# dmosopt/dmosopt

Measured on AMD Instinct MI355X. Metric: MO-ASMO epoch time (GP fit + 200-gen NSGA2), ZDT1 d=30, lower is better.
Workload: dtype fp32; 1 GPU; model=GPR-Matern52 surrogate + NSGA2, global_batch=200, parallelism=replicated-moea+sharded-gp dp1, population_size=200, archive_size=300

## Files before the change

dmosopt_amd/ops/hip/moea_device.h:

```cpp
#pragma once

#include "common.h"
#include <math.h>

__device__ __forceinline__ void sbx_children(float a, float b, float beta,
                                             float lo, float hi, float* c1,
                                             float* c2) {
  const float x1 = 0.5f * fmaf(-beta, a, fmaf(beta, b, a + b));
  const float x2 = 0.5f * fmaf(beta, a, fmaf(-beta, b, a + b));
  *c1 = fminf(fmaxf(x1, lo), hi);
  *c2 = fminf(fmaxf(x2, lo), hi);
}

__device__ __forceinline__ float mutated_child(float p, float delta, float lo,
                                               float hi) {
  const float v = fmaf(hi - lo, delta, p);
  return fminf(fmaxf(v, lo), hi);
}

template <typename PoolIdx>
__device__ __forceinline__ void variation_event_gene(
    const float* __restrict__ src, const PoolIdx* pool_row,
    const long long* __restrict__ ci, const long long* __restrict__ mi,
    const long long* __restrict__ p1, const long long* __restrict__ p2,
    const long long* __restrict__ im, const float* __restrict__ di_c,
    const float* __restrict__ di_m, const float* __restrict__ lo,
    const float* __restrict__ hi, float* __restrict__ out, int ev, int g,
    int C, int d, float mutation_rate, unsigned long long seed_sbx,
    unsigned long long seed_mut) {
  if (ev < C) {
    long long r1 = p1[ev], r2 = p2[ev];
    if (pool_row) { r1 = (long long)pool_row[r1]; r2 = (long long)pool_row[r2]; }
    const float a = src[r1 * d + g];
    const float b = src[r2 * d + g];
    const Philox4 r = philox4x32(seed_sbx, (unsigned long long)ev * d + g);
    const float u = u01(r.c0);
    const float e = 1.f / (di_c[g] + 1.f);
    const float beta = (u <= 0.5f) ? __powf(2.f * u, e)
                                   : __powf(1.f / (2.f * (1.f - u)), e);
    float c1, c2;
    sbx_children(a, b, beta, lo[g], hi[g], &c1, &c2);
    out[ci[2 * ev] * d + g] = c1;
    out[ci[2 * ev + 1] * d + g] = c2;
  } else {
    const int m = ev - C;
    long long r0 = im[m];
    if (pool_row) r0 = (long long)pool_row[r0];
    const float p = src[r0 * d + g];
    const Philox4 ph =
        philox4x32(seed_mut ^ 0x5deece66dULL, (unsigned long long)m * d + g);
    const float u = u01(ph.c0);
    const float e = 1.f / (di_m[g] + 1.f);
    const float delta = (u < mutation_rate)
                            ? __powf(2.f * u, e) - 1.f
                            : 1.f - __powf(2.f * (1.f - u), e);
    out[mi[m] * d + g] = mutated_child(p, delta, lo[g], hi[g]);
  }
}

__device__ __forceinline__ void crowding_gaps(const float* vals,
                                              const int* idxs, float* out,
                                              int N, int tid, int nthreads) {
  const float l = vals[0];
  const float h = vals[N - 1];
  float s = h - l;
  if (!(s > 0.f) || !isfinite(s)) s = 1.f;
  for (int i = tid; i < N; i += nthreads) {
    float d = (i == 0 || i == N - 1) ? 1.f : (vals[i + 1] - vals[i - 1]) / s;
    if (isnan(d)) d = 0.f;
    out[idxs[i]] = d;
  }
}

__device__ __forceinline__ void crowding_sort_gaps(float* vals, int* idxs,
                                                   float* out, int N,
                                                   int npow2, int tid,
                                                   int nthreads,
                                                   bool active = true) {
  for (int ksz = 2; ksz <= npow2; ksz <<= 1) {
    for (int jsz = ksz >> 1; jsz > 0; jsz >>= 1) {
      for (int i = tid; active && i < npow2; i += nthreads) {
        const int ixj = i ^ jsz;
        if (ixj > i) {
          const bool up = ((i & ksz) == 0);
          const bool swap = up ? (vals[i] > vals[ixj]) : (vals[i] < vals[ixj]);
          if (swap) {
            float tv = vals[i]; vals[i] = vals[ixj]; vals[ixj] = tv;
            int tixx = idxs[i]; idxs[i] = idxs[ixj]; idxs[ixj] = tixx;
          }
        }
      }
      __syncthreads();
    }
  }
  if (active) crowding_gaps(vals, idxs, out, N, tid, nthreads);
}

__device__ __forceinline__ long long rank_crowd_key(long long rank, float d) {
  if (isnan(d)) d = 0.f;
  const unsigned int b = __float_as_uint(d);
  const unsigned int asc = (b & 0x80000000u) ? ~b : (b | 0x80000000u);
  return (rank << 32) | (long long)(0xFFFFFFFFu - asc);
}

__device__ __forceinline__ void key_idx_sort(long long* keys, int* idxs, int M,
                                             int tid, int nthreads) {
  for (int k = 2; k <= M; k <<= 1) {
    for (int j = k >> 1; j > 0; j >>= 1) {
      for (int i = tid; i < M; i += nthreads) {
        const int ixj = i ^ j;
        if (ixj > i) {
          const bool up = ((i & k) == 0);
          const long long ka = keys[i], kb = keys[ixj];
          const int ia = idxs[i], ib = idxs[ixj];
          const bool gt = (ka > kb) || (ka == kb && ia > ib);
          if (gt == up) {
            keys[i] = kb; keys[ixj] = ka;
            idxs[i] = ib; idxs[ixj] = ia;
          }
        }
      }
      __syncthreads();
    }
  }
}
```

dmosopt_amd/ops/hip/moea_ops.hip:

```cpp

#include "common.h"
#include "launchers.h"
#include "moea_device.h"
#include <math.h>
#include <algorithm>

#define TOUR_TPB 256
#define TOUR_NMAX 2048

template <int TPB, bool COUNT>
__device__ __forceinline__ const int* tournament_order(
    const long long* __restrict__ rank, long long* key, int* idx, float* gkey,
    int* unsorted, int N, int npow2, float log1mp, unsigned long long seed) {
  const int tid = threadIdx.x;
  if (tid == 0) { unsorted[0] = 0; unsorted[1] = 0; }
  __syncthreads();
  for (int i = tid; i < npow2; i += TPB) {
    key[i] = (i < N) ? (rank[i] * (long long)N + i) : 0x7FFFFFFFFFFFFFFFLL;
    idx[i] = i;
    if (i + 1 < N && rank[i] > rank[i + 1]) atomicOr(&unsorted[0], 1);
  }
  __syncthreads();
  if (unsorted[0])
  for (int ks = 2; ks <= npow2; ks <<= 1) {
    for (int js = ks >> 1; js > 0; js >>= 1) {
      for (int i = tid; i < npow2; i += TPB) {
        const int ixj = i ^ js;
        if (ixj > i) {
          const bool up = ((i & ks) == 0);
          if (up ? (key[i] > key[ixj]) : (key[i] < key[ixj])) {
            long long tk = key[i]; key[i] = key[ixj]; key[ixj] = tk;
            int ti = idx[i]; idx[i] = idx[ixj]; idx[ixj] = ti;
          }
        }
      }
      __syncthreads();
    }
  }
  for (int i = tid; i < npow2; i += TPB) {
    if (i < N) {
      Philox4 r = philox4x32(seed, (unsigned long long)i);
      const float u = u01(r.c0);
      gkey[i] = (float)i * log1mp - logf(-logf(u));
    } else {
      gkey[i] = -INFINITY;
    }
  }
  __syncthreads();
  if (COUNT) {
    int* sel = (int*)key;
    bool tie = false;
    for (int i = tid; i < N; i += TPB) {
      const float gi = gkey[i];
      int pos = 0;
#pragma unroll 8
      for (int j = 0; j < N; ++j) {
        const float gj = gkey[j];
        pos += (gj > gi || (gj == gi && j < i)) ? 1 : 0;
        tie |= (gj == gi && j != i);
      }
      tie |= (gi != gi);
      sel[pos] = idx[i];
    }
    if (tie) atomicOr(&unsorted[1], 1);
    __syncthreads();
    if (!unsorted[1]) return sel;
  }
  for (int ks = 2; ks <= npow2; ks <<= 1) {
    for (int js = ks >> 1; js > 0; js >>= 1) {
      for (int i = tid; i < npow2; i += TPB) {
        const int ixj = i ^ js;
        if (ixj > i) {
          const bool up = ((i & ks) == 0);
          if (up ? (gkey[i] < gkey[ixj]) : (gkey[i] > gkey[ixj])) {
            float tg = gkey[i]; gkey[i] = gkey[ixj]; gkey[ixj] = tg;
            int ti = idx[i]; idx[i] = idx[ixj]; idx[ixj] = ti;
          }
        }
      }
      __syncthreads();
    }
  }
  return idx;
}

template <int TPB>
__global__ __launch_bounds__(TPB) void tournament_kernel(
    const float* __restrict__ population, const long long* __restrict__ rank,
    float* __restrict__ pool, long long* __restrict__ pool_idx, int N, int d,
    int poolsize, int npow2, float log1mp, unsigned long long seed) {
  extern __shared__ char sh_raw[];
  long long* key = (long long*)sh_raw;
  int* idx = (int*)(key + npow2);
  float* gkey = (float*)(idx + npow2);
  __shared__ int unsorted[2];
  const int tid = threadIdx.x;
  tournament_order<TPB, false>(rank, key, idx, gkey, unsorted, N, npow2,
                               log1mp, seed);
  for (int j = tid; j < poolsize; j += TPB) pool_idx[j] = idx[j];
  __syncthreads();
  for (long long t = tid; t < (long long)poolsize * d; t += TPB) {
    const int r = (int)(t / d), c = (int)(t % d);
    pool[t] = population[(long long)idx[r] * d + c];
  }
}

template <int TPB>
__global__ __launch_bounds__(TPB) void spawn_fused_kernel(
    const float* __restrict__ population, const long long* __restrict__ rank,
    int N, int d, int npow2, float log1mp, unsigned long long seed_t,
    const long long* __restrict__ ci, const long long* __restrict__ mi,
    const long long* __restrict__ p1, const long long* __restrict__ p2,
    const long long* __restrict__ im, const float* __restrict__ di_c,
    const float* __restrict__ di_m, const float* __restrict__ lo,
    const float* __restrict__ hi, float* __restrict__ out, int C, int M,
    float mutation_rate, unsigned long long seed_sbx,
    unsigned long long seed_mut) {
  extern __shared__ char sh_raw[];
  long long* key = (long long*)sh_raw;
  int* idx = (int*)(key + npow2);
  float* gkey = (float*)(idx + npow2);
  __shared__ int unsorted[2];
  const int* pool_row = tournament_order<TPB, true>(
      rank, key, idx, gkey, unsorted, N, npow2, log1mp, seed_t);
  const int total = (C + M) * d;
  for (int t = blockIdx.x * TPB + threadIdx.x; t < total; t += gridDim.x * TPB)
    variation_event_gene<int>(population, pool_row, ci, mi, p1, p2, im, di_c, di_m,
                              lo, hi, out, t / d, t % d, C, d, mutation_rate,
                              seed_sbx, seed_mut);
}

extern "C" int launch_tournament(const float* population, const long long* rank,
                                 float* pool, long long* pool_idx, int N,
                                 int d, int poolsize, float log1mp,
                                 unsigned long long seed, hipStream_t stream) {
  int npow2 = 1;
  while (npow2 < N) npow2 <<= 1;
  if (npow2 > TOUR_NMAX) return -1;
  const size_t lds = (size_t)npow2 * (8 + 4 + 4);
  if (npow2 > 512)
    hipLaunchKernelGGL(tournament_kernel<1024>, dim3(1), dim3(1024), lds,
                       stream, population, rank, pool, pool_idx, N, d,
                       poolsize, npow2, log1mp, seed);
  else
    hipLaunchKernelGGL(tournament_kernel<TOUR_TPB>, dim3(1), dim3(TOUR_TPB),
                       lds, stream, population, rank, pool, pool_idx, N, d,
                       poolsize, npow2, log1mp, seed);
  return 0;
}

extern "C" int launch_spawn_fused(
    const float* population, const long long* rank, int N, int d, int poolsize,
    float log1mp, unsigned long long seed_t, const long long* ci,
    const long long* mi, const long long* p1, const long long* p2,
    const long long* im, const float* di_c, const float* di_m, const float* lo,
    const float* hi, float* out, int C, int M, float mutation_rate,
    unsigned long long seed_sbx, unsigned long long seed_mut,
    hipStream_t stream) {
  int npow2 = 1;
  while (npow2 < N) npow2 <<= 1;
  if (npow2 > TOUR_NMAX || poolsize > N) return -1;
  const size_t lds = (size_t)npow2 * (8 + 4 + 4);
  const long long total = (long long)(C + M) * d;
  const int tpb = npow2 > 512 ? 1024 : TOUR_TPB;
  const int blocks =
      (int)std::min<long long>(64, std::max<long long>(1, (total + 2 * tpb - 1) / (2 * tpb)));
  if (npow2 > 512)
    hipLaunchKernelGGL(spawn_fused_kernel<1024>, dim3(blocks), dim3(1024), lds,
                       stream, population, rank, N, d, npow2, log1mp, seed_t,
                       ci, mi, p1, p2, im, di_c, di_m, lo, hi, out, C, M,
                       mutation_rate, seed_sbx, seed_mut);
  else
    hipLaunchKernelGGL(spawn_fused_kernel<TOUR_TPB>, dim3(blocks), dim3(TOUR_TPB),
                       lds, stream, population, rank, N, d, npow2, log1mp,
                       seed_t, ci, mi, p1, p2, im, di_c, di_m, lo, hi, out, C,
                       M, mutation_rate, seed_sbx, seed_mut);
  return 0;
}

#define SELF_TPB 512
#define SELF_CG 2

struct SelLds {
  size_t keys, sidx, cvals, ys, db, fmask, ndom, rank, perdim, cross, ctrl, total;
};

static __host__ __device__ inline SelLds sel_lds(int N, int m, int ng,
                                                 int npow2) {
  const size_t W = (N + 31) / 32;
  SelLds L;
  size_t o = 0;
  L.keys = o;   o += (size_t)npow2 * 8;
  L.sidx = o;   o += (size_t)npow2 * 4;
  L.cvals = o;  o += (size_t)SELF_CG * npow2 * 8;
  L.ys = o;     o += (size_t)N * m * 4;
  L.db = o;     o += (size_t)N * W * 4;
  L.fmask = o;  o += W * 4;
  L.ndom = o;   o += (size_t)N * 4;
  L.rank = o;   o += (size_t)N * 4;
  L.perdim = o; o += (size_t)N * m * 4;
  L.cross = o;  o += (size_t)((ng + 31) / 32) * 4;
  L.ctrl = o;   o += 16;
  L.total = o;
  return L;
}

template <int M>
__global__ void dom_bits_pair_kernel(const float* __restrict__ y_gen,
                                     const float* __restrict__ pop_obj,
                                     unsigned int* __restrict__ Dbits, int ng,
                                     int N, int m, int W) {
  const int idx = blockIdx.x * blockDim.x + threadIdx.x;
  if (idx >= N * W) return;
  const int j = idx / W, w = idx % W;
  const int mm = M > 0 ? M : m;
  const float* yj = (j < ng) ? y_gen + (size_t)j * mm
                             : pop_obj + (size_t)(j - ng) * mm;
  float cj[M > 0 ? M : 1];
  if (M > 0) {
#pragma unroll
    for (int t = 0; t < M; ++t) cj[t] = yj[t];
  }
  unsigned int bits = 0;
  const int i0 = w * 32;
  const int iend = min(32, N - i0);
  for (int b = 0; b < iend; ++b) {
    const int i = i0 + b;
    const float* yi = (i < ng) ? y_gen + (size_t)i * mm
                               : pop_obj + (size_t)(i - ng) * mm;
    bool le = true, lt = false;
    if (M > 0) {
#pragma unroll
      for (int t = 0; t < M; ++t) {
        const float a = yi[t];
        le &= (a <= cj[t]);
        lt |= (a < cj[t]);
      }
    } else {
      for (int t = 0; t < m; ++t) {
        const float a = yi[t], c = yj[t];
        le &= (a <= c);
        lt |= (a < c);
      }
    }
    if (le && lt && i != j) bits |= (1u << b);
  }
  Dbits[idx] = bits;
}

__global__ __launch_bounds__(SELF_TPB) void nsga2_select_fused_kernel(
    const float* __restrict__ x_gen, const float* __restrict__ y_gen,
    const float* __restrict__ pop_parm, const float* __restrict__ pop_obj,
    const unsigned int* __restrict__ Dbits, int ng, int np, int d, int m, int keep, int npow2,
    const long long* __restrict__ c_idx, int n_cross,
    float* __restrict__ parm_o, float* __restrict__ obj_o,
    long long* __restrict__ rank_o, long long* __restrict__ perm,
    long long* __restrict__ succ_cross, long long* __restrict__ succ_mut) {
  extern __shared__ char sh_raw[];
  const int N = ng + np, W = (N + 31) / 32;
  const SelLds L = sel_lds(N, m, ng, npow2);
  long long* keys = (long long*)(sh_raw + L.keys);
  int* sidx = (int*)(sh_raw + L.sidx);
  float* Ys = (float*)(sh_raw + L.ys);
  unsigned int* Db = (unsigned int*)(sh_raw + L.db);
  unsigned int* fmask = (unsigned int*)(sh_raw + L.fmask);
  int* n_dom = (int*)(sh_raw + L.ndom);
  int* rank = (int*)(sh_raw + L.rank);
  float* per_dim = (float*)(sh_raw + L.perdim);
  unsigned int* is_cross = (unsigned int*)(sh_raw + L.cross);
  int* ctrl = (int*)(sh_raw + L.ctrl);
  const int tid = threadIdx.x;

  for (int t = tid; t < N * m; t += SELF_TPB)
    Ys[t] = (t < ng * m) ? y_gen[t] : pop_obj[t - ng * m];
  for (int w = tid; w < (ng + 31) / 32; w += SELF_TPB) is_cross[w] = 0u;
  if (tid == 0) { ctrl[1] = 0; ctrl[2] = 0; }
  __syncthreads();

  for (int t = tid; t < N * W; t += SELF_TPB) Db[t] = Dbits[t];
  __syncthreads();
  for (int j = tid; j < N; j += SELF_TPB) {
    int cnt = 0;
    for (int w = 0; w < W; ++w) cnt += __popc(Db[j * W + w]);
    n_dom[j] = cnt;
    rank[j] = 0;
  }
  __syncthreads();

  int ranked = 0;
  for (int k = 0; ranked < N && k <= N; ++k) {
    if (tid == 0) ctrl[0] = 0;
    for (int w = tid; w < W; w += SELF_TPB) fmask[w] = 0u;
    __syncthreads();
    for (int j = tid; j < N; j += SELF_TPB) {
      if (n_dom[j] == 0) {
        rank[j] = k;
        n_dom[j] = -1;
        atomicOr(&fmask[j >> 5], 1u << (j & 31));
        atomicAdd(&ctrl[0], 1);
      }
    }
    __syncthreads();
    const int fs = ctrl[0];
    if (fs == 0) break;
    ranked += fs;
    if (ranked >= keep) {
      for (int j = tid; j < N; j += SELF_TPB)
        if (n_dom[j] > 0) rank[j] = k + 1;
      break;
    }
    for (int j = tid; j < N; j += SELF_TPB) {
      if (n_dom[j] <= 0) continue;
      int dec = 0;
#pragma unroll 4
      for (int w = 0; w < W; ++w) dec += __popc(Db[j * W + w] & fmask[w]);
      n_dom[j] -= dec;
    }
    __syncthreads();
  }
  __syncthreads();

  {
    constexpr int GT = SELF_TPB / SELF_CG;
    const int grp = tid / GT, gtid = tid % GT;
    float* gv = (float*)(sh_raw + L.cvals) + (size_t)grp * 2 * npow2;
    int* gi = (int*)(gv + npow2);
    for (int o0 = 0; o0 < m; o0 += SELF_CG) {
      const int o = o0 + grp;
      const bool active = o < m;
      for (int i = gtid; active && i < npow2; i += GT) {
        gv[i] = (i < N) ? Ys[i * m + o] : INFINITY;
        gi[i] = i;
      }
      __syncthreads();
      crowding_sort_gaps(gv, gi, per_dim + (size_t)(active ? o : 0) * N, N,
                         npow2, gtid, GT, active);
      __syncthreads();
    }
  }

  for (int i = tid; i < npow2; i += SELF_TPB) {
    if (i < N) {
      float acc = 0.f;
      for (int o = 0; o < m; ++o) acc += per_dim[(size_t)o * N + i];
      keys[i] = rank_crowd_key((long long)rank[i], acc);
      sidx[i] = i;
    } else {
      keys[i] = 0x7FFFFFFFFFFFFFFFLL;
      sidx[i] = 0x7FFFFFFF;
    }
  }
  __syncthreads();
  key_idx_sort(keys, sidx, npow2, tid, SELF_TPB);

  const int P = min(keep, N);
  for (int r = tid; r < P; r += SELF_TPB) {
    const int src = sidx[r];
    perm[r] = (long long)src;
    rank_o[r] = (long long)rank[src];
  }
  for (int t = tid; t < P * m; t += SELF_TPB)
    obj_o[t] = Ys[sidx[t / m] * m + t % m];
#pragma unroll 4
  for (int t = tid; t < P * d; t += SELF_TPB) {
    const int src = sidx[t / d], c = t % d;
    parm_o[t] = (src < ng) ? x_gen[(size_t)src * d + c]
                           : pop_parm[(size_t)(src - ng) * d + c];
  }
  if (succ_cross == nullptr) return;
  for (int i = tid; i < n_cross; i += SELF_TPB) {
    const int s = (int)c_idx[i];
    if (s >= 0 && s < ng) atomicOr(&is_cross[s >> 5], 1u << (s & 31));
  }
  __syncthreads();
  int lc = 0, lm = 0;
  for (int r = tid; r < P; r += SELF_TPB) {
    const int e = sidx[r];
    if (e < ng) {
      if (is_cross[e >> 5] & (1u << (e & 31))) ++lc;
      else ++lm;
    }
  }
  if (lc) atomicAdd(&ctrl[1], lc);
  if (lm) atomicAdd(&ctrl[2], lm);
  __syncthreads();
  if (tid == 0) {
    atomicAdd((unsigned long long*)succ_cross,
              (unsigned long long)(ctrl[1] / 2));
    atomicAdd((unsigned long long*)succ_mut, (unsigned long long)ctrl[2]);
  }
}

extern "C" int nsga2_select_fused_fits(int ng, int np, int m) {
  const int N = ng + np;
  if (ng < 1 || np < 1 || m < 1 || N > 2048) return 0;
  int npow2 = 1;
  while (npow2 < N) npow2 <<= 1;
  return sel_lds(N, m, ng, npow2).total <= 144 * 1024 ? 1 : 0;
}

extern "C" int launch_nsga2_select_fused(
    const float* x_gen, const float* y_gen, const float* pop_parm,
    const float* pop_obj, int ng, int np, int d, int m, int keep,
    const long long* c_idx, int n_cross, unsigned int* dbits_scratch,
    float* parm_o, float* obj_o, long long* rank_o, long long* perm,
    long long* succ_cross, long long* succ_mut, hipStream_t stream) {
  if (!nsga2_select_fused_fits(ng, np, m)) return -1;
  const int N = ng + np;
  int npow2 = 1;
  while (npow2 < N) npow2 <<= 1;
  const size_t lds = sel_lds(N, m, ng, npow2).total;
  static bool attr_set = false;
  if (!attr_set) {
    (void)hipFuncSetAttribute((const void*)nsga2_select_fused_kernel,
                              hipFuncAttributeMaxDynamicSharedMemorySize,
                              144 * 1024);
    attr_set = true;
  }
  const int W = (N + 31) / 32;
  const int blocks = (N * W + 255) / 256;
  if (m == 2)
    hipLaunchKernelGGL(dom_bits_pair_kernel<2>, dim3(blocks), dim3(256), 0,
                       stream, y_gen, pop_obj, dbits_scratch, ng, N, m, W);
  else if (m == 3)
    hipLaunchKernelGGL(dom_bits_pair_kernel<3>, dim3(blocks), dim3(256), 0,
                       stream, y_gen, pop_obj, dbits_scratch, ng, N, m, W);
  else
    hipLaunchKernelGGL(dom_bits_pair_kernel<0>, dim3(blocks), dim3(256), 0,
                       stream, y_gen, pop_obj, dbits_scratch, ng, N, m, W);
  hipLaunchKernelGGL(nsga2_select_fused_kernel, dim3(1), dim3(SELF_TPB), lds,
                     stream, x_gen, y_gen, pop_parm, pop_obj,
                     (const unsigned int*)dbits_scratch, ng, np, d, m, keep,
                     npow2, c_idx, n_cross, parm_o, obj_o, rank_o, perm,
                     succ_cross, succ_mut);
  return 0;
}

__global__ void survivor_count_kernel(const long long* __restrict__ perm,
                                      const long long* __restrict__ c_idx,
                                      int n_perm, int n_cross, int n_children,
                                      long long* __restrict__ succ_cross,
                                      long long* __restrict__ succ_mut) {
  __shared__ unsigned int is_cross[(2048 + 31) / 32];
  __shared__ int cnt_c, cnt_m;
  const int tid = threadIdx.x;
  const int words = (n_children + 31) / 32;
  for (int w = tid; w < words; w += blockDim.x) is_cross[w] = 0u;
  if (tid == 0) { cnt_c = 0; cnt_m = 0; }
  __syncthreads();
  for (int i = tid; i < n_cross; i += blockDim.x) {
    const int s = (int)c_idx[i];
    atomicOr(&is_cross[s >> 5], 1u << (s & 31));
  }
  __syncthreads();
  int lc = 0, lm = 0;
  for (int i = tid; i < n_perm; i += blockDim.x) {
    const long long e = perm[i];
    if (e < n_children) {
      if (is_cross[(int)(e >> 5)] & (1u << ((int)e & 31))) ++lc;
      else ++lm;
    }
  }
  atomicAdd(&cnt_c, lc);
  atomicAdd(&cnt_m, lm);
  __syncthreads();
  if (tid == 0) {
    atomicAdd((unsigned long long*)succ_cross, (unsigned long long)(cnt_c / 2));
    atomicAdd((unsigned long long*)succ_mut, (unsigned long long)cnt_m);
  }
}

extern "C" int launch_survivor_count(const long long* perm,
                                     const long long* c_idx, int n_perm,
                                     int n_cross, int n_children,
                                     long long* succ_cross,
                                     long long* succ_mut,
                                     hipStream_t stream) {
  if (n_children > 2048) return -1;
  hipLaunchKernelGGL(survivor_count_kernel, dim3(1), dim3(256), 0, stream,
                     perm, c_idx, n_perm, n_cross, n_children, succ_cross,
                     succ_mut);
  return 0;
}

__global__ void pack_rank_crowd_kernel(const long long* __restrict__ rank,
                                       const float* __restrict__ crowd,
                                       long long* __restrict__ key, int N) {
  const int i = blockIdx.x * blockDim.x + threadIdx.x;
  if (i >= N) return;
  float d = crowd[i];
  if (!(d >= 0.f)) d = 0.f;
  if (isinf(d)) d = 3.4028235e38f;
  unsigned int bits = __float_as_uint(d);
  key[i] = (rank[i] << 32) | (long long)(0x7FFFFFFFu - bits);
}

extern "C" void launch_pack_rank_crowd(const long long* rank,
                                       const float* crowd, long long* key,
                                       int N, hipStream_t stream) {
  hipLaunchKernelGGL(pack_rank_crowd_kernel, dim3((N + 255) / 256), dim3(256),
                     0, stream, rank, crowd, key, N);
}

__global__ void gather3_kernel(const float* __restrict__ parm,
                               const float* __restrict__ obj,
                               const long long* __restrict__ rank,
                               const long long* __restrict__ perm,
                               float* __restrict__ parm_o,
                               float* __restrict__ obj_o,
                               long long* __restrict__ rank_o, int pop, int d,
                               int m) {
  const long long t = (long long)blockIdx.x * blockDim.x + threadIdx.x;
  const long long total = (long long)pop * (d + m + 1);
  if (t >= total) return;
  const int r = (int)(t / (d + m + 1));
  const int c = (int)(t % (d + m + 1));
  const long long src = perm[r];
  if (c < d) parm_o[(long long)r * d + c] = parm[src * d + c];
  else if (c < d + m) obj_o[(long long)r * m + (c - d)] = obj[src * m + (c - d)];
  else rank_o[r] = rank[src];
}

extern "C" void launch_gather3(const float* parm, const float* obj,
                               const long long* rank, const long long* perm,
                               float* parm_o, float* obj_o, long long* rank_o,
                               int pop, int d, int m, hipStream_t stream) {
  const long long total = (long long)pop * (d + m + 1);
  hipLaunchKernelGGL(gather3_kernel, dim3((int)((total + 255) / 256)),
                     dim3(256), 0, stream, parm, obj, rank, perm, parm_o,
                     obj_o, rank_o, pop, d, m);
}

#define RCS_TPB 1024

__global__ __launch_bounds__(RCS_TPB) void rank_crowd_sort_kernel(
    const long long* __restrict__ rank, const float* __restrict__ crowd,
    long long* __restrict__ perm, int N, int pop) {
  extern __shared__ char sh[];
  long long* keys = (long long*)sh;
  int* idxs = (int*)(keys + 0);
  int M = 1;
  while (M < N) M <<= 1;
  idxs = (int*)(keys + M);
  const int tid = threadIdx.x;

  for (int i = tid; i < M; i += RCS_TPB) {
    if (i < N) {
      keys[i] = rank_crowd_key((long long)rank[i], crowd[i]);
      idxs[i] = i;
    } else {
      keys[i] = 0x7FFFFFFFFFFFFFFFLL;
      idxs[i] = 0x7FFFFFFF;
    }
  }
  __syncthreads();
  key_idx_sort(keys, idxs, M, tid, RCS_TPB);
  for (int i = tid; i < pop && i < N; i += RCS_TPB)
    perm[i] = (long long)idxs[i];
}

extern "C" int launch_rank_crowd_sort(const long long* rank,
                                      const float* crowd, long long* perm,
                                      int N, int pop, hipStream_t stream) {
  int M = 1;
  while (M < N) M <<= 1;
  const size_t lds = (size_t)M * (sizeof(long long) + sizeof(int));
  if (lds > 144 * 1024) return -1;
  static bool attr_set = false;
  if (!attr_set) {
    hipFuncSetAttribute((const void*)rank_crowd_sort_kernel,
                        hipFuncAttributeMaxDynamicSharedMemorySize, 144 * 1024);
    attr_set = true;
  }
  hipLaunchKernelGGL(rank_crowd_sort_kernel, dim3(1), dim3(RCS_TPB), lds,
                     stream, rank, crowd, perm, N, pop);
  return 0;
}

__global__ void smpso_velocity_kernel(
    const float* __restrict__ position,
    const float* __restrict__ velocity,
    const float* __restrict__ leader1,
    const float* __restrict__ leader2,
    const float* __restrict__ xlb, const float* __restrict__ xub,
    float* __restrict__ out, int n, int d, float w, float a1, float a2,
    float chi) {
  const long long t = (long long)blockIdx.x * blockDim.x + threadIdx.x;
  if (t >= (long long)n * d) return;
  const int k = (int)(t % d);
  const float p = position[t];
  const float v = chi * (w * velocity[t] + a1 * (leader1[k] - p) +
                         a2 * (leader2[k] - p));
  const float delta = 0.5f * (xub[k] - xlb[k]);
  out[t] = fminf(fmaxf(v, -delta), delta);
}

extern "C" void launch_smpso_velocity(const float* position,
                                      const float* velocity,
                                      const float* leader1,
                                      const float* leader2, const float* xlb,
                                      const float* xub, float* out, int n,
                                      int d, float w, float a1, float a2,
                                      float chi, hipStream_t stream) {
  const long long total = (long long)n * d;
  hipLaunchKernelGGL(smpso_velocity_kernel,
                     dim3((unsigned)((total + 255) / 256)), dim3(256), 0,
                     stream, position, velocity, leader1, leader2, xlb, xub,
                     out, n, d, w, a1, a2, chi);
}

__global__ void cat_rows_kernel(const float* __restrict__ a,
                                const float* __restrict__ b,
                                float* __restrict__ out, long long na_elems,
                                long long total_elems) {
  const long long i = (long long)blockIdx.x * blockDim.x + threadIdx.x;
  if (i >= total_elems) return;
  out[i] = (i < na_elems) ? a[i] : b[i - na_elems];
}

extern "C" void launch_cat_rows(const float* a, const float* b, float* out,
                                long long na_elems, long long total_elems,
                                hipStream_t stream) {
  hipLaunchKernelGGL(cat_rows_kernel,
                     dim3((int)((total_elems + 255) / 256)), dim3(256), 0,
                     stream, a, b, out, na_elems, total_elems);
}

__global__ void colsum_kernel(const float* __restrict__ per_dim,
                              float* __restrict__ out, int m, int N) {
  const int i = blockIdx.x * blockDim.x + threadIdx.x;
  if (i >= N) return;
  float acc = 0.f;
  for (int j = 0; j < m; ++j) acc += per_dim[(long long)j * N + i];
  out[i] = acc;
}

extern "C" void launch_colsum(const float* per_dim, float* out, int m, int N,
                              hipStream_t stream) {
  hipLaunchKernelGGL(colsum_kernel, dim3((N + 255) / 256), dim3(256), 0,
                     stream, per_dim, out, m, N);
}
```

dmosopt_amd/ops/hip/nsga3.hip:

```cpp

#include "launchers.h"
#include "moea_device.h"

#include <limits.h>

#define NSGA3_MAX_N 4096
#define NSGA3_MAX_H 2048
#define NSGA3_MAX_M 16

#define NSGA3_L 0
#define NSGA3_NP 1
#define NSGA3_NS 2
#define NSGA3_R 3

#define NSGA3_NICHE_TPB 1024
#define NSGA3_NICHE_SLOTS (NSGA3_MAX_N / NSGA3_NICHE_TPB)
#define NSGA3_LDS_LIMIT (144 * 1024)

static size_t nsga3_niche_lds(int N, int H) {
  size_t M = 1;
  while (M < (size_t)N) M <<= 1;
  return 12 * M + 12 * (size_t)H;
}

extern "C" int nsga3_select_fits(int N, int H, int m) {
  return N >= 1 && N <= NSGA3_MAX_N && H >= 1 && H <= NSGA3_MAX_H && m >= 1 &&
         m <= NSGA3_MAX_M && nsga3_niche_lds(N, H) <= NSGA3_LDS_LIMIT;
}

__global__ __launch_bounds__(1024) void nsga3_normalize_kernel(
    const float* __restrict__ Y, const long long* __restrict__ rank, int N,
    int m, int K, int H, float* __restrict__ ideal, float* __restrict__ scale,
    int* __restrict__ ctrl, int* __restrict__ rho) {
  __shared__ int cum[2][NSGA3_MAX_N];
  __shared__ int s_ctrl[4];
  __shared__ float s_z[NSGA3_MAX_M], s_fmax[NSGA3_MAX_M];
  __shared__ int s_ext[NSGA3_MAX_M];
  __shared__ double s_E[NSGA3_MAX_M][NSGA3_MAX_M + 1];
  const int tid = threadIdx.x, nt = blockDim.x;
  const int lane = tid & 63, wave = tid >> 6;

  for (int i = tid; i < N; i += nt) cum[0][i] = 0;
  for (int h = tid; h < H; h += nt) rho[h] = 0;
  __syncthreads();
  for (int i = tid; i < N; i += nt) {
    const long long r = rank[i];
    if (r >= 0 && r < N) atomicAdd(&cum[0][(int)r], 1);
  }
  __syncthreads();
  int src = 0;
  for (int off = 1; off < N; off <<= 1) {
    for (int i = tid; i < N; i += nt)
      cum[src ^ 1][i] = cum[src][i] + (i >= off ? cum[src][i - off] : 0);
    __syncthreads();
    src ^= 1;
  }
  for (int i = tid; i < N; i += nt) {
    const int before = i ? cum[src][i - 1] : 0;
    if (cum[src][i] >= K && before < K) {
      s_ctrl[NSGA3_L] = i;
      s_ctrl[NSGA3_NP] = before;
      s_ctrl[NSGA3_NS] = cum[src][i];
      s_ctrl[NSGA3_R] = K - before;
    }
  }
  __syncthreads();
  const int l = s_ctrl[NSGA3_L];

  if (wave < m) {
    float mn = INFINITY, mx = -INFINITY;
    for (int i = lane; i < N; i += WAVE_SIZE) {
      const long long r = rank[i];
      const float v = Y[(long long)i * m + wave];
      if (r <= l) mn = fminf(mn, v);
      if (r == 0) mx = fmaxf(mx, v);
    }
    for (int off = 32; off > 0; off >>= 1) {
      mn = fminf(mn, __shfl_xor(mn, off, WAVE_SIZE));
      mx = fmaxf(mx, __shfl_xor(mx, off, WAVE_SIZE));
    }
    if (lane == 0) {
      s_z[wave] = mn;
      s_fmax[wave] = mx - mn;
    }
  }
  __syncthreads();

  if (wave < m) {
    float bv = INFINITY;
    int bi = INT_MAX;
    for (int i = lane; i < N; i += WAVE_SIZE) {
      if (rank[i] != 0) continue;
      float v = -INFINITY;
      for (int k = 0; k < m; ++k) {
        const float t = Y[(long long)i * m + k] - s_z[k];
        v = fmaxf(v, k == wave ? t : t / 1e-6f);
      }
      if (v < bv || bi == INT_MAX) { bv = v; bi = i; }
    }
    for (int off = 32; off > 0; off >>= 1) {
      const float ov = __shfl_xor(bv, off, WAVE_SIZE);
      const int oi = __shfl_xor(bi, off, WAVE_SIZE);
      if (oi != INT_MAX && (bi == INT_MAX || ov < bv || (ov == bv && oi < bi))) {
        bv = ov;
        bi = oi;
      }
    }
    if (lane == 0) s_ext[wave] = bi;
  }
  __syncthreads();

  if (tid == 0) {
    bool ok = true;
    for (int a = 0; a < m && ok; ++a) {
      if (s_ext[a] < 0 || s_ext[a] >= N) ok = false;
      for (int b = 0; b < a && ok; ++b) ok = s_ext[a] != s_ext[b];
    }
    if (ok) {
      for (int j = 0; j < m; ++j) {
        for (int k = 0; k < m; ++k)
          s_E[j][k] = (double)(Y[(long long)s_ext[j] * m + k] - s_z[k]);
        s_E[j][m] = 1.0;
      }
      for (int c = 0; c < m && ok; ++c) {
        int p = c;
        for (int r = c + 1; r < m; ++r)
          if (fabs(s_E[r][c]) > fabs(s_E[p][c])) p = r;
        if (s_E[p][c] == 0.0) { ok = false; break; }
        if (p != c)
          for (int k = c; k <= m; ++k) {
            const double t = s_E[c][k]; s_E[c][k] = s_E[p][k]; s_E[p][k] = t;
          }
        for (int r = c + 1; r < m; ++r) {
          const double f = s_E[r][c] / s_E[c][c];
          for (int k = c; k <= m; ++k) s_E[r][k] -= f * s_E[c][k];
        }
      }
      if (ok) {
        for (int c = m - 1; c >= 0; --c) {
          double acc = s_E[c][m];
          for (int k = c + 1; k < m; ++k) acc -= s_E[c][k] * s_E[k][m];
          s_E[c][m] = acc / s_E[c][c];
        }
        for (int j = 0; j < m; ++j) {
          const double a = s_E[j][m];
          if (!(isfinite(a) && a > 0.0)) ok = false;
        }
      }
    }
    for (int j = 0; j < m; ++j) {
      float s = ok ? (float)(1.0 / s_E[j][m]) : s_fmax[j];
      if (!(s >= 1e-6f)) s = 1.f;
      scale[j] = s;
      ideal[j] = s_z[j];
    }
    for (int q = 0; q < 4; ++q) ctrl[q] = s_ctrl[q];
  }
}

#define NSGA3_TILE 256
#define NSGA3_LPR 16

__global__ __launch_bounds__(256) void nsga3_associate_kernel(
    const float* __restrict__ Y, const long long* __restrict__ rank,
    const float* __restrict__ ideal, const float* __restrict__ scale,
    const int* __restrict__ ctrl, const float* __restrict__ Z, int N, int H,
    int m, long long* __restrict__ niche, float* __restrict__ dist,
    int* __restrict__ rho) {
  __shared__ float zt[NSGA3_MAX_M][NSGA3_TILE];
  const int tid = threadIdx.x;
  const int sub = tid & (NSGA3_LPR - 1);
  const int row = blockIdx.x * (256 / NSGA3_LPR) + tid / NSGA3_LPR;
  const int l = ctrl[NSGA3_L];
  const long long r = row < N ? rank[row] : (long long)INT_MAX;
  const bool act = r <= l;

  float yp[NSGA3_MAX_M];
#pragma unroll
  for (int k = 0; k < NSGA3_MAX_M; ++k)
    yp[k] = (act && k < m) ? (Y[(long long)row * m + k] - ideal[k]) / scale[k]
                           : 0.f;

  float bd = INFINITY;
  int bh = INT_MAX;
  for (int h0 = 0; h0 < H; h0 += NSGA3_TILE) {
    __syncthreads();
    if (h0 + tid < H) {
      const float* z = Z + (long long)(h0 + tid) * m;
      float s = 0.f;
      for (int k = 0; k < m; ++k) s = fmaf(z[k], z[k], s);
      const float nrm = sqrtf(s);
      for (int k = 0; k < m; ++k) zt[k][tid] = z[k] / nrm;
    }
    __syncthreads();
    const int nh = min(NSGA3_TILE, H - h0);
    if (act) {
      for (int hh = sub; hh < nh; hh += NSGA3_LPR) {
        float dot = 0.f;
#pragma unroll
        for (int k = 0; k < NSGA3_MAX_M; ++k)
          if (k < m) dot = fmaf(yp[k], zt[k][hh], dot);
        float d2 = 0.f;
#pragma unroll
        for (int k = 0; k < NSGA3_MAX_M; ++k)
          if (k < m) {
            const float e = fmaf(-dot, zt[k][hh], yp[k]);
            d2 = fmaf(e, e, d2);
          }
        const float d = sqrtf(d2);
        if (d < bd) { bd = d; bh = h0 + hh; }
      }
    }
  }
  for (int off = NSGA3_LPR / 2; off > 0; off >>= 1) {
    const float od = __shfl_xor(bd, off, WAVE_SIZE);
    const int oh = __shfl_xor(bh, off, WAVE_SIZE);
    if (od < bd || (od == bd && oh < bh)) { bd = od; bh = oh; }
  }
  if (sub == 0 && row < N) {
    if (act) {
      if (bh >= H) bh = 0;
      niche[row] = bh;
      dist[row] = bd;
      if (r < l) atomicAdd(&rho[bh], 1);
    } else {
      niche[row] = -1;
      dist[row] = INFINITY;
    }
  }
}

__global__ __launch_bounds__(NSGA3_NICHE_TPB) void nsga3_niche_kernel(
    const float* __restrict__ x_gen, const float* __restrict__ pop_parm,
    const float* __restrict__ Y, const long long* __restrict__ rank,
    const long long* __restrict__ niche, const float* __restrict__ dist,
    const int* __restrict__ ctrl, const int* __restrict__ rho,
    const long long* __restrict__ dir_prio,
    const long long* __restrict__ row_prio, int ng, int np, int d, int m, int H,
    int K, float* __restrict__ parm_o, float* __restrict__ obj_o,
    long long* __restrict__ rank_o, long long* __restrict__ perm) {
  extern __shared__ long long nsga3_lds[];
  const int tid = threadIdx.x, nt = blockDim.x;
  const int N = ng + np;
  int M = 1;
  while (M < N) M <<= 1;
  long long* keys = nsga3_lds;
  unsigned long long* first = (unsigned long long*)(keys + M);
  int* idxs = (int*)(first + H);
  int* start = idxs + M;
  const int l = ctrl[NSGA3_L];

  for (int h = tid; h < H; h += nt) {
    first[h] = ~0ull;
    start[h] = 0;
  }
  __syncthreads();
  for (int i = tid; i < N; i += nt)
    if (rank[i] == l)
      atomicMin(&first[niche[i]],
                ((unsigned long long)__float_as_uint(dist[i]) << 32) |
                    (unsigned int)i);
  __syncthreads();
  for (int i = tid; i < M; i += nt) {
    long long key = LLONG_MAX;
    if (i < N && rank[i] == l) {
      const int h = (int)niche[i];
      const bool is_first = rho[h] == 0 && (unsigned int)first[h] == (unsigned int)i;
      key = ((long long)h << 32) | (is_first ? 0ll : 1ll << 31) | row_prio[i];
    }
    keys[i] = key;
    idxs[i] = i;
  }
  __syncthreads();
  key_idx_sort(keys, idxs, M, tid, nt);
  for (int p = tid; p < M; p += nt)
    if (keys[p] != LLONG_MAX) {
      const int h = (int)(keys[p] >> 32);
      if (p == 0 || (int)(keys[p - 1] >> 32) != h) start[h] = p;
    }
  __syncthreads();
  long long nk[NSGA3_NICHE_SLOTS];
  int ni[NSGA3_NICHE_SLOTS];
#pragma unroll
  for (int q = 0; q < NSGA3_NICHE_SLOTS; ++q) {
    const int p = tid + q * nt;
    nk[q] = LLONG_MAX;
    ni[q] = p;
    if (p < M) {
      const int i = idxs[p];
      ni[q] = i;
      if (keys[p] != LLONG_MAX) {
        const int h = (int)(keys[p] >> 32);
        nk[q] = (1ll << 40) + (long long)(rho[h] + p - start[h]) * H + dir_prio[h];
      } else if (i < N && rank[i] < l) {
        nk[q] = rank[i] * N + i;
      }
    }
  }
  __syncthreads();
#pragma unroll
  for (int q = 0; q < NSGA3_NICHE_SLOTS; ++q) {
    const int p = tid + q * nt;
    if (p < M) { keys[p] = nk[q]; idxs[p] = ni[q]; }
  }
  __syncthreads();
  key_idx_sort(keys, idxs, M, tid, nt);

  for (int p = tid; p < K; p += nt) {
    const int i = idxs[p];
    perm[p] = i;
    rank_o[p] = rank[i];
  }
  for (int e = tid; e < K * d; e += nt) {
    const int i = idxs[e / d], c = e % d;
    parm_o[e] = i < ng ? x_gen[(long long)i * d + c]
                       : pop_parm[(long long)(i - ng) * d + c];
  }
  for (int e = tid; e < K * m; e += nt)
    obj_o[e] = Y[(long long)idxs[e / m] * m + e % m];
}

extern "C" int launch_nsga3_select(
    const float* x_gen, const float* pop_parm, const float* Y,
    const long long* rank, const float* Z, const long long* dir_prio,
    const long long* row_prio, int ng, int np, int d, int m, int H, int K,
    int* ctrl, int* rho, float* ideal, float* scale, long long* niche,
    float* dist, float* parm_o, float* obj_o, long long* rank_o,
    long long* perm, hipStream_t stream) {
  const int N = ng + np;
  if (!nsga3_select_fits(N, H, m) || K < 1 || K > N || d < 1) return -1;
  hipLaunchKernelGGL(nsga3_normalize_kernel, dim3(1), dim3(1024), 0, stream, Y,
                     rank, N, m, K, H, ideal, scale, ctrl, rho);
  hipLaunchKernelGGL(nsga3_associate_kernel,
                     dim3((N + 256 / NSGA3_LPR - 1) / (256 / NSGA3_LPR)),
                     dim3(256), 0, stream, Y, rank, ideal, scale, ctrl, Z, N, H,
                     m, niche, dist, rho);
  static bool attr_set = false;
  if (!attr_set) {
    (void)hipFuncSetAttribute((const void*)nsga3_niche_kernel,
                              hipFuncAttributeMaxDynamicSharedMemorySize,
                              NSGA3_LDS_LIMIT);
    attr_set = true;
  }
  hipLaunchKernelGGL(nsga3_niche_kernel, dim3(1), dim3(NSGA3_NICHE_TPB),
                     nsga3_niche_lds(N, H), stream, x_gen,
                     pop_parm, Y, rank, niche, dist, ctrl, rho, dir_prio,
                     row_prio, ng, np, d, m, H, K, parm_o, obj_o, rank_o, perm);
  return 0;
}
```

dmosopt_amd/ops/hip/pareto.hip:

```cpp

#include "common.h"
#include "launchers.h"
#include "moea_device.h"
#include <math.h>

#define PTILE 32
#define PTPB 256

__global__ void dominance_matrix_kernel(const float* __restrict__ Y,
                                        int* __restrict__ D,
                                        int N, int m) {
  extern __shared__ float lds[];
  float* yi = lds;
  float* yj = lds + PTILE * m;
  const int ti = blockIdx.y * PTILE;
  const int tj = blockIdx.x * PTILE;
  for (int idx = threadIdx.x; idx < PTILE * m; idx += PTPB) {
    const int r = idx / m, c = idx % m;
    yi[idx] = (ti + r < N) ? Y[(ti + r) * m + c] : 0.f;
    yj[idx] = (tj + r < N) ? Y[(tj + r) * m + c] : 0.f;
  }
  __syncthreads();
  const int ty = threadIdx.x / 16, tx = threadIdx.x % 16;
#pragma unroll
  for (int sy = 0; sy < 2; ++sy)
#pragma unroll
    for (int sx = 0; sx < 2; ++sx) {
      const int li = ty * 2 + sy, lj = tx * 2 + sx;
      const int gi = ti + li, gj = tj + lj;
      if (gi >= N || gj >= N) continue;
      int cnt = 0;
      for (int k = 0; k < m; ++k)
        cnt += (yi[li * m + k] <= yj[lj * m + k]) ? 1 : 0;
      D[(long long)gi * N + gj] = cnt;
    }
}

extern "C" void launch_dominance_matrix(const float* Y, int* D, int N, int m,
                                        hipStream_t stream) {
  dim3 grid((N + PTILE - 1) / PTILE, (N + PTILE - 1) / PTILE);
  size_t lds_bytes = 2 * PTILE * m * sizeof(float);
  hipLaunchKernelGGL(dominance_matrix_kernel, grid, dim3(PTPB), lds_bytes,
                     stream, Y, D, N, m);
}

template <int M>
__global__ void dom_bits_kernel(const float* __restrict__ Y,
                                unsigned int* __restrict__ Dbits,
                                int N, int m, int W) {
  const long long idx = (long long)blockIdx.x * blockDim.x + threadIdx.x;
  if (idx >= (long long)N * W) return;
  const int j = (int)(idx / W), w = (int)(idx % W);
  unsigned int bits = 0;
  const int i0 = w * 32;
  const int iend = min(32, N - i0);
  if (M > 0) {
    float cj[M > 0 ? M : 1];
#pragma unroll
    for (int t = 0; t < M; ++t) cj[t] = Y[j * M + t];
    for (int b = 0; b < iend; ++b) {
      const int i = i0 + b;
      bool le = true, lt = false;
#pragma unroll
      for (int t = 0; t < M; ++t) {
        const float a = Y[i * M + t];
        le &= (a <= cj[t]);
        lt |= (a < cj[t]);
      }
      if (le && lt && i != j) bits |= (1u << b);
    }
  } else {
    for (int b = 0; b < iend; ++b) {
      const int i = i0 + b;
      if (i == j) continue;
      bool le = true, lt = false;
      for (int t = 0; t < m; ++t) {
        const float a = Y[i * m + t], c = Y[j * m + t];
        le &= (a <= c);
        lt |= (a < c);
      }
      if (le && lt) bits |= (1u << b);
    }
  }
  Dbits[idx] = bits;
}

#define PEELB_TPB 256

__global__ __launch_bounds__(PEELB_TPB) void peel_bits_kernel(
    const unsigned int* __restrict__ Dbits, int* __restrict__ rank, int N,
    int W) {
  extern __shared__ char sh_raw[];
  unsigned int* Db = (unsigned int*)sh_raw;
  unsigned int* fmask = Db + (size_t)N * W;
  int* n_dom = (int*)(fmask + W);
  int* ctrl = n_dom + N;
  const int tid = threadIdx.x;

  for (int i = tid; i < N * W; i += PEELB_TPB) Db[i] = Dbits[i];
  if (tid == 0) ctrl[1] = N;
  __syncthreads();
  for (int j = tid; j < N; j += PEELB_TPB) {
    int c = 0;
    for (int w = 0; w < W; ++w) c += __popc(Db[j * W + w]);
    n_dom[j] = c;
  }
  __syncthreads();

  for (int k = 0; ctrl[1] > 0 && k <= N; ++k) {
    if (tid == 0) ctrl[0] = 0;
    for (int w = tid; w < W; w += PEELB_TPB) fmask[w] = 0u;
    __syncthreads();
    for (int j = tid; j < N; j += PEELB_TPB) {
      if (n_dom[j] == 0) {
        rank[j] = k;
        n_dom[j] = -1;
        atomicOr(&fmask[j >> 5], 1u << (j & 31));
        atomicAdd(&ctrl[0], 1);
      }
    }
    __syncthreads();
    const int fs = ctrl[0];
    if (fs == 0) break;
    for (int j = tid; j < N; j += PEELB_TPB) {
      if (n_dom[j] <= 0) continue;
      int dec = 0;
      for (int w = 0; w < W; ++w) dec += __popc(Db[j * W + w] & fmask[w]);
      n_dom[j] -= dec;
    }
    __syncthreads();
    if (tid == 0) ctrl[1] -= fs;
    __syncthreads();
  }
}

#define LAUNCH_DOM_BITS(blocks_, stream_, Y_, D_, N_, m_, W_)                  do {                                                                           if (m_ == 2)                                                                   hipLaunchKernelGGL(dom_bits_kernel<2>, dim3(blocks_), dim3(256), 0,                               stream_, Y_, D_, N_, m_, W_);                          else if (m_ == 3)                                                              hipLaunchKernelGGL(dom_bits_kernel<3>, dim3(blocks_), dim3(256), 0,                               stream_, Y_, D_, N_, m_, W_);                          else if (m_ == 5)                                                              hipLaunchKernelGGL(dom_bits_kernel<5>, dim3(blocks_), dim3(256), 0,                               stream_, Y_, D_, N_, m_, W_);                          else                                                                           hipLaunchKernelGGL(dom_bits_kernel<0>, dim3(blocks_), dim3(256), 0,                               stream_, Y_, D_, N_, m_, W_);                        } while (0)

extern "C" int launch_peel_bits(const float* Y, unsigned int* Dbits_scratch,
                                int* rank, int N, int m, hipStream_t stream) {
  const int W = (N + 31) / 32;
  const size_t lds = ((size_t)N * W + W) * sizeof(unsigned int) +
                     (N + 2) * sizeof(int);
  if (lds > 144 * 1024) return -1;
  static bool attr_set = false;
  if (!attr_set) {
    hipFuncSetAttribute((const void*)peel_bits_kernel,
                        hipFuncAttributeMaxDynamicSharedMemorySize, 144 * 1024);
    attr_set = true;
  }
  const long long total = (long long)N * W;
  LAUNCH_DOM_BITS(((int)((total + 255) / 256)), stream, Y, Dbits_scratch, N,
                  m, W);
  hipLaunchKernelGGL(peel_bits_kernel, dim3(1), dim3(PEELB_TPB), lds, stream,
                     Dbits_scratch, rank, N, W);
  return 0;
}

#include <hip/hip_cooperative_groups.h>

__global__ __launch_bounds__(256) void coop_peel_bits_kernel(
    const unsigned int* __restrict__ Dbits,
    unsigned int* __restrict__ fmask,
    int* __restrict__ n_dom,
    int* __restrict__ ctrl,
    int* __restrict__ rank,
    int N, int W, int stop) {
  cooperative_groups::grid_group grid = cooperative_groups::this_grid();
  const int gtid = blockIdx.x * blockDim.x + threadIdx.x;
  const int gsize = gridDim.x * blockDim.x;

  for (int j = gtid; j < N; j += gsize) {
    int c = 0;
    const unsigned int* row = Dbits + (size_t)j * W;
    for (int w = 0; w < W; ++w) c += __popc(row[w]);
    n_dom[j] = c;
    rank[j] = 0;
  }
  for (int w = gtid; w < 3 * W; w += gsize) fmask[w] = 0u;
  if (gtid == 0) ctrl[0] = 0;
  grid.sync();
  for (int j = gtid; j < N; j += gsize) {
    if (n_dom[j] == 0) {
      n_dom[j] = -1;
      atomicOr(&fmask[j >> 5], 1u << (j & 31));
      atomicAdd(&ctrl[0], 1);
    }
  }
  grid.sync();

  int prev = -1;
  for (int k = 0; k < N; ++k) {
    const int total = ctrl[0];
    if (total >= N || total == prev) break;
    if (total >= stop) {
      for (int j = gtid; j < N; j += gsize)
        if (n_dom[j] >= 0) rank[j] = k + 1;
      break;
    }
    prev = total;
    const unsigned int* rd = fmask + (size_t)(k % 3) * W;
    unsigned int* wr = fmask + (size_t)((k + 1) % 3) * W;
    unsigned int* cl = fmask + (size_t)((k + 2) % 3) * W;
    for (int w = gtid; w < W; w += gsize) cl[w] = 0u;
    for (int j = gtid; j < N; j += gsize) {
      if (n_dom[j] <= 0) continue;
      int dec = 0;
      const unsigned int* row = Dbits + (size_t)j * W;
      for (int w = 0; w < W; ++w) dec += __popc(row[w] & rd[w]);
      if (dec) {
        const int nd = n_dom[j] - dec;
        if (nd == 0) {
          rank[j] = k + 1;
          n_dom[j] = -1;
          atomicOr(&wr[j >> 5], 1u << (j & 31));
          atomicAdd(&ctrl[0], 1);
        } else {
          n_dom[j] = nd;
        }
      }
    }
    grid.sync();
  }
}

extern "C" int launch_coop_peel(const float* Y, unsigned int* Dbits,
                                unsigned int* fmask, int* n_dom, int* ctrl,
                                int* rank, int N, int m, int stop,
                                hipStream_t stream) {
  const int W = (N + 31) / 32;
  if (stop <= 0 || stop > N) stop = N;
  static int coop_ok = -1;
  if (coop_ok < 0) {
    int dev = 0, attr = 0;
    hipGetDevice(&dev);
    hipDeviceGetAttribute(&attr, hipDeviceAttributeCooperativeLaunch, dev);
    coop_ok = attr ? 1 : 0;
  }
  if (!coop_ok) return -1;
  static int max_blocks = -1;
  if (max_blocks < 0) {
    int per_cu = 0;
    hipOccupancyMaxActiveBlocksPerMultiprocessor(
        &per_cu, (const void*)coop_peel_bits_kernel, 256, 0);
    hipDeviceProp_t prop;
    int dev = 0;
    hipGetDevice(&dev);
    hipGetDeviceProperties(&prop, dev);
    max_blocks = per_cu * prop.multiProcessorCount;
    if (max_blocks < 1) max_blocks = 1;
  }
  const long long total = (long long)N * W;
  LAUNCH_DOM_BITS(((int)((total + 255) / 256)), stream, Y, Dbits, N, m, W);
  int blocks = (N + 255) / 256;
  if (blocks > max_blocks) blocks = max_blocks;
  void* args[] = {(void*)&Dbits, (void*)&fmask, (void*)&n_dom,
                  (void*)&ctrl, (void*)&rank, (void*)&N, (void*)&W,
                  (void*)&stop};
  const hipError_t err = hipLaunchCooperativeKernel(
      (const void*)coop_peel_bits_kernel, dim3(blocks), dim3(256),
      args, 0, stream);
  return err == hipSuccess ? 0 : -1;
}

#define CROWD_TPB 256

template <int TPB>
__global__ __launch_bounds__(TPB) void crowding_kernel(
    const float* __restrict__ Y,
    float* __restrict__ out,
    int N, int m, int npow2) {
  extern __shared__ float sh[];
  float* vals = sh;
  int* idxs = (int*)(sh + npow2);
  const int j = blockIdx.x;

  for (int i = threadIdx.x; i < npow2; i += TPB) {
    vals[i] = (i < N) ? Y[i * m + j] : INFINITY;
    idxs[i] = i;
  }
  __syncthreads();

  crowding_sort_gaps(vals, idxs, out + (long long)j * N, N, npow2,
                     threadIdx.x, TPB);
}

extern "C" void launch_crowding(const float* Y, float* out, int N, int m,
                                hipStream_t stream) {
  int npow2 = 1;
  while (npow2 < N) npow2 <<= 1;
  size_t lds_bytes = npow2 * (sizeof(float) + sizeof(int));
  if (npow2 > 512)
    hipLaunchKernelGGL(crowding_kernel<1024>, dim3(m), dim3(1024), lds_bytes,
                       stream, Y, out, N, m, npow2);
  else
    hipLaunchKernelGGL(crowding_kernel<CROWD_TPB>, dim3(m), dim3(CROWD_TPB),
                       lds_bytes, stream, Y, out, N, m, npow2);
}
```

Measured before the change: 62.46 ms_per_epoch.

## Run intra-wave bitonic sort stages with register shuffles instead of LDS barriers

Replaces the several block-wide bitonic sort loops (crowding, tournament order, key/index sorts, NSGA3 niching) with one shared helper. Stages whose compare distance is 64 or less run inside a wavefront using __shfl_xor on values held in registers, and only the larger distances go through LDS with __syncthreads. The aim is to cut the barrier count and LDS traffic of the small sorts that run every generation. It relies on each 64-element chunk mapping to a single wave, and the descending and tie-break comparators have to behave the same as before.

```diff
diff --git a/dmosopt_amd/ops/hip/moea_device.h b/dmosopt_amd/ops/hip/moea_device.h
--- a/dmosopt_amd/ops/hip/moea_device.h
+++ b/dmosopt_amd/ops/hip/moea_device.h
@@ -58,6 +58,78 @@
   }
 }
 
+struct SwapAsc {
+  template <typename K>
+  __device__ __forceinline__ bool operator()(K a, int, K b, int, bool up) const {
+    return up ? (a > b) : (a < b);
+  }
+};
+struct SwapDesc {
+  template <typename K>
+  __device__ __forceinline__ bool operator()(K a, int, K b, int, bool up) const {
+    return up ? (a < b) : (a > b);
+  }
+};
+struct SwapKeyIdx {
+  template <typename K>
+  __device__ __forceinline__ bool operator()(K ka, int ia, K kb, int ib,
+                                             bool up) const {
+    const bool gt = (ka > kb) || (ka == kb && ia > ib);
+    return gt == up;
+  }
+};
+
+template <int NT, typename K, typename Swap>
+__device__ __forceinline__ void bitonic_wave_run(K* keys, int* idxs, int M,
+                                                 int tid, bool active,
+                                                 int k_first, int k_last,
+                                                 Swap swap) {
+  for (int i = tid; active && (i & ~63) < M; i += NT) {
+    const bool in = i < M;
+    K k = in ? keys[i] : K(0);
+    int x = in ? idxs[i] : 0;
+    for (int ksz = k_first; ksz <= k_last; ksz <<= 1) {
+      const bool up = ((i & ksz) == 0);
+      for (int jsz = min(ksz >> 1, 32); jsz > 0; jsz >>= 1) {
+        const K pk = __shfl_xor(k, jsz);
+        const int px = __shfl_xor(x, jsz);
+        const bool lower = ((i & jsz) == 0);
+        const bool sw = lower ? swap(k, x, pk, px, up) : swap(pk, px, k, x, up);
+        if (sw) { k = pk; x = px; }
+      }
+    }
+    if (in) { keys[i] = k; idxs[i] = x; }
+  }
+}
+
+template <int NT, typename K, typename Swap>
+__device__ __forceinline__ void bitonic_sort_pairs(K* keys, int* idxs, int M,
+                                                   bool active, Swap swap) {
+  static_assert(NT % 64 == 0, "a 64-element block must belong to one wave");
+  const int tid = threadIdx.x % NT;
+  bitonic_wave_run<NT>(keys, idxs, M, tid, active, 2, min(M, 64), swap);
+  __syncthreads();
+  for (int ksz = 128; ksz <= M; ksz <<= 1) {
+    for (int jsz = ksz >> 1; jsz >= 64; jsz >>= 1) {
+      for (int i = tid; active && i < M; i += NT) {
+        const int ixj = i ^ jsz;
+        if (ixj > i) {
+          const bool up = ((i & ksz) == 0);
+          const K ka = keys[i], kb = keys[ixj];
+          const int ia = idxs[i], ib = idxs[ixj];
+          if (swap(ka, ia, kb, ib, up)) {
+            keys[i] = kb; keys[ixj] = ka;
+            idxs[i] = ib; idxs[ixj] = ia;
+          }
+        }
+      }
+      __syncthreads();
+    }
+    bitonic_wave_run<NT>(keys, idxs, M, tid, active, ksz, ksz, swap);
+    __syncthreads();
+  }
+}
+
 __device__ __forceinline__ void crowding_gaps(const float* vals,
                                               const int* idxs, float* out,
                                               int N, int tid, int nthreads) {
@@ -72,28 +144,13 @@
   }
 }
 
+template <int NT>
 __device__ __forceinline__ void crowding_sort_gaps(float* vals, int* idxs,
                                                    float* out, int N,
-                                                   int npow2, int tid,
-                                                   int nthreads,
+                                                   int npow2,
                                                    bool active = true) {
-  for (int ksz = 2; ksz <= npow2; ksz <<= 1) {
-    for (int jsz = ksz >> 1; jsz > 0; jsz >>= 1) {
-      for (int i = tid; active && i < npow2; i += nthreads) {
-        const int ixj = i ^ jsz;
-        if (ixj > i) {
-          const bool up = ((i & ksz) == 0);
-          const bool swap = up ? (vals[i] > vals[ixj]) : (vals[i] < vals[ixj]);
-          if (swap) {
-            float tv = vals[i]; vals[i] = vals[ixj]; vals[ixj] = tv;
-            int tixx = idxs[i]; idxs[i] = idxs[ixj]; idxs[ixj] = tixx;
-          }
-        }
-      }
-      __syncthreads();
-    }
-  }
-  if (active) crowding_gaps(vals, idxs, out, N, tid, nthreads);
+  bitonic_sort_pairs<NT>(vals, idxs, npow2, active, SwapAsc());
+  if (active) crowding_gaps(vals, idxs, out, N, threadIdx.x % NT, NT);
 }
 
 __device__ __forceinline__ long long rank_crowd_key(long long rank, float d) {
@@ -103,24 +160,8 @@
   return (rank << 32) | (long long)(0xFFFFFFFFu - asc);
 }
 
-__device__ __forceinline__ void key_idx_sort(long long* keys, int* idxs, int M,
-                                             int tid, int nthreads) {
-  for (int k = 2; k <= M; k <<= 1) {
-    for (int j = k >> 1; j > 0; j >>= 1) {
-      for (int i = tid; i < M; i += nthreads) {
-        const int ixj = i ^ j;
-        if (ixj > i) {
-          const bool up = ((i & k) == 0);
-          const long long ka = keys[i], kb = keys[ixj];
-          const int ia = idxs[i], ib = idxs[ixj];
-          const bool gt = (ka > kb) || (ka == kb && ia > ib);
-          if (gt == up) {
-            keys[i] = kb; keys[ixj] = ka;
-            idxs[i] = ib; idxs[ixj] = ia;
-          }
-        }
-      }
-      __syncthreads();
-    }
-  }
+template <int NT>
+__device__ __forceinline__ void key_idx_sort(long long* keys, int* idxs,
+                                             int M) {
+  bitonic_sort_pairs<NT>(keys, idxs, M, true, SwapKeyIdx());
 }
diff --git a/dmosopt_amd/ops/hip/moea_ops.hip b/dmosopt_amd/ops/hip/moea_ops.hip
--- a/dmosopt_amd/ops/hip/moea_ops.hip
+++ b/dmosopt_amd/ops/hip/moea_ops.hip
@@ -22,21 +22,7 @@
   }
   __syncthreads();
   if (unsorted[0])
-  for (int ks = 2; ks <= npow2; ks <<= 1) {
-    for (int js = ks >> 1; js > 0; js >>= 1) {
-      for (int i = tid; i < npow2; i += TPB) {
-        const int ixj = i ^ js;
-        if (ixj > i) {
-          const bool up = ((i & ks) == 0);
-          if (up ? (key[i] > key[ixj]) : (key[i] < key[ixj])) {
-            long long tk = key[i]; key[i] = key[ixj]; key[ixj] = tk;
-            int ti = idx[i]; idx[i] = idx[ixj]; idx[ixj] = ti;
-          }
-        }
-      }
-      __syncthreads();
-    }
-  }
+    bitonic_sort_pairs<TPB>(key, idx, npow2, true, SwapAsc());
   for (int i = tid; i < npow2; i += TPB) {
     if (i < N) {
       Philox4 r = philox4x32(seed, (unsigned long long)i);
@@ -66,21 +52,7 @@
     __syncthreads();
     if (!unsorted[1]) return sel;
   }
-  for (int ks = 2; ks <= npow2; ks <<= 1) {
-    for (int js = ks >> 1; js > 0; js >>= 1) {
-      for (int i = tid; i < npow2; i += TPB) {
-        const int ixj = i ^ js;
-        if (ixj > i) {
-          const bool up = ((i & ks) == 0);
-          if (up ? (gkey[i] < gkey[ixj]) : (gkey[i] > gkey[ixj])) {
-            float tg = gkey[i]; gkey[i] = gkey[ixj]; gkey[ixj] = tg;
-            int ti = idx[i]; idx[i] = idx[ixj]; idx[ixj] = ti;
-          }
-        }
-      }
-      __syncthreads();
-    }
-  }
+  bitonic_sort_pairs<TPB>(gkey, idx, npow2, true, SwapDesc());
   return idx;
 }
 
@@ -333,8 +305,8 @@
         gi[i] = i;
       }
       __syncthreads();
-      crowding_sort_gaps(gv, gi, per_dim + (size_t)(active ? o : 0) * N, N,
-                         npow2, gtid, GT, active);
+      crowding_sort_gaps<GT>(gv, gi, per_dim + (size_t)(active ? o : 0) * N, N,
+                             npow2, active);
       __syncthreads();
     }
   }
@@ -351,7 +323,7 @@
     }
   }
   __syncthreads();
-  key_idx_sort(keys, sidx, npow2, tid, SELF_TPB);
+  key_idx_sort<SELF_TPB>(keys, sidx, npow2);
 
   const int P = min(keep, N);
   for (int r = tid; r < P; r += SELF_TPB) {
@@ -554,7 +526,7 @@
     }
   }
   __syncthreads();
-  key_idx_sort(keys, idxs, M, tid, RCS_TPB);
+  key_idx_sort<RCS_TPB>(keys, idxs, M);
   for (int i = tid; i < pop && i < N; i += RCS_TPB)
     perm[i] = (long long)idxs[i];
 }
diff --git a/dmosopt_amd/ops/hip/nsga3.hip b/dmosopt_amd/ops/hip/nsga3.hip
--- a/dmosopt_amd/ops/hip/nsga3.hip
+++ b/dmosopt_amd/ops/hip/nsga3.hip
@@ -272,7 +272,7 @@
     idxs[i] = i;
   }
   __syncthreads();
-  key_idx_sort(keys, idxs, M, tid, nt);
+  key_idx_sort<NSGA3_NICHE_TPB>(keys, idxs, M);
   for (int p = tid; p < M; p += nt)
     if (keys[p] != LLONG_MAX) {
       const int h = (int)(keys[p] >> 32);
@@ -304,7 +304,7 @@
     if (p < M) { keys[p] = nk[q]; idxs[p] = ni[q]; }
   }
   __syncthreads();
-  key_idx_sort(keys, idxs, M, tid, nt);
+  key_idx_sort<NSGA3_NICHE_TPB>(keys, idxs, M);
 
   for (int p = tid; p < K; p += nt) {
     const int i = idxs[p];
diff --git a/dmosopt_amd/ops/hip/pareto.hip b/dmosopt_amd/ops/hip/pareto.hip
--- a/dmosopt_amd/ops/hip/pareto.hip
+++ b/dmosopt_amd/ops/hip/pareto.hip
@@ -280,8 +280,7 @@
   }
   __syncthreads();
 
-  crowding_sort_gaps(vals, idxs, out + (long long)j * N, N, npow2,
-                     threadIdx.x, TPB);
+  crowding_sort_gaps<TPB>(vals, idxs, out + (long long)j * N, N, npow2);
 }
 
 extern "C" void launch_crowding(const float* Y, float* out, int N, int m,
```

New measurement: 64.55 ms_per_epoch. 1.03x slower.
